# Funatiq/cuclark

Measured on AMD Instinct MI355X. Metric: Mreads/sec (10M x 150bp, k=31), higher is better.
Workload: dtype u64

## Files before the change

cuclark_amd/csrc/mic_device.h:

```cpp
#ifndef MIC_DEVICE_H
#define MIC_DEVICE_H

#include "mic_internal.h"

__device__ __forceinline__ uint32_t bperm(int src_lane, uint32_t v) {
  return (uint32_t)__builtin_amdgcn_ds_bpermute(src_lane << 2, (int)v);
}

template <int CTRL>
__device__ __forceinline__ uint32_t quad_perm(uint32_t v) {
  return (uint32_t)__builtin_amdgcn_update_dpp(0, (int)v, CTRL, 0xF, 0xF, true);
}
#define QP_BCAST0 0x00
#define QP_BCAST1 0x55
#define QP_BCAST3 0xFF
#define QP_XOR1 0xB1
#define QP_XOR2 0x4E

__device__ __forceinline__ uint64_t revcomp_bits(uint64_t x, int k) {
  uint32_t rh = __builtin_bitreverse32((uint32_t)x), rl = __builtin_bitreverse32((uint32_t)(x >> 32));
  rh = ((rh >> 1) & 0x55555555u) | ((rh << 1) & ~0x55555555u);
  rl = ((rl >> 1) & 0x55555555u) | ((rl << 1) & ~0x55555555u);
  return (((uint64_t)~rh << 32) | (uint32_t)~rl) >> (64 - 2 * k);
}

__device__ __forceinline__ uint64_t canonical(uint64_t kmer, int k) {
  uint64_t rc = revcomp_bits(kmer, k);
  return kmer < rc ? kmer : rc;
}

#ifndef MIC_HASH_LITE
#define MIC_HASH_LITE 2
#endif
#ifndef MIC_CHEAP_HASH
#define MIC_CHEAP_HASH 1
#endif
__device__ __forceinline__ uint32_t mmer_order_key_canon(uint64_t u) {
#if MIC_CHEAP_HASH
  const uint32_t hi = (uint32_t)(u >> 32);
  uint32_t h = (uint32_t)u * 0x9E3779B1u ^ (__umul24(hi ^ (hi >> 24), 0xEBCA77u) + 0x27D4EB2Fu);
#else
  uint32_t h = (uint32_t)u * 0x9E3779B1u ^ ((uint32_t)(u >> 32) * 0x85EBCA77u + 0x27D4EB2Fu);
#endif
#if MIC_HASH_LITE & 1
  h *= 0x2C1B3C6Du;
#else
  h ^= h >> 15; h *= 0x2C1B3C6Du;
#endif
  return h;
}

__device__ __forceinline__ uint32_t mmer_order_key(uint64_t x, int m) { return mmer_order_key_canon(canonical(x, m)); }

__device__ __forceinline__ uint32_t mslot_of_key(uint32_t min_key, uint32_t n_slots) {
#if MIC_CHEAP_HASH
  return __umulhi(min_key * 0xC2B2AE3Du, n_slots);
#else
  uint32_t z = min_key * 0xC2B2AE3Du;
  z ^= z >> 15; z *= 0x165667B1u;
  return __umulhi(z, n_slots);
#endif
}

__device__ __forceinline__ uint32_t mslot_of_kmer(uint64_t kmer, int k, int m, uint32_t n_slots) {
  const uint64_t mask = (1ULL << (2 * m)) - 1;
  uint32_t best = 0xFFFFFFFFu;
  for (int j = 0; j + m <= k; ++j) {
    uint32_t h = mmer_order_key((kmer >> (2 * (k - m - j))) & mask, m);
    best = h < best ? h : best;
  }
  return mslot_of_key(best, n_slots);
}

#define MIC_S_CAP 6
#define MIC_S_NEXT 0x100u

#ifndef MIC_S_MOD
#define MIC_S_MOD 1
#endif
__host__ __device__ __forceinline__ int s_tlen(int k, int m) {
  int t = m;
#if MIC_S_MOD
  const int w = k - m + 1;
  while (t - w >= 7) t -= w;
#endif
  return t;
}
__device__ __forceinline__ uint32_t s_torder(uint64_t tv) {
  uint32_t h = __umul24((uint32_t)tv & 0xFFFFFFu, 0x9E3779u) + 0x27D4EB2Fu;
  const uint32_t hi = (uint32_t)(tv >> 24);
  if (hi) h += hi * 0x85EBCA77u + (uint32_t)(tv >> 56) * 0xC2B2AE3Du;
  return h;
}
__device__ __forceinline__ uint32_t s_torder24(uint32_t tv) { return __umul24(tv, 0x9E3779u) + 0x27D4EB2Fu; }
__device__ __forceinline__ uint32_t swap_comp_pairs(uint32_t a, uint32_t b) {
#if defined(__HIP_DEVICE_COMPILE__)
  return (uint32_t)__builtin_amdgcn_bitop3_b32(a, b, 0x55555555u, 0x1B);
#else
  return ~((a & 0x55555555u) | (b & ~0x55555555u));
#endif
}
__device__ __forceinline__ uint32_t revcomp_bits32(uint32_t x, int t) {
#if defined(__HIP_DEVICE_COMPILE__)
  const uint32_t br = __builtin_bitreverse32(x);
  const uint32_t b = (__builtin_constant_p(t) && t < 16) ? br >> (31 - 2 * t) : (br << 1) >> (32 - 2 * t);
  return swap_comp_pairs(br >> (33 - 2 * t), b) & (t >= 16 ? 0xFFFFFFFFu : (1u << (2 * t)) - 1u);
#else
  uint32_t r = __builtin_bitreverse32(x) >> (32 - 2 * t);
  r = ((r >> 1) & 0x55555555u) | ((r << 1) & ~0x55555555u);
  return ~r & (t >= 16 ? 0xFFFFFFFFu : (1u << (2 * t)) - 1u);
#endif
}
template <typename F>
__device__ __forceinline__ void s_sampled(uint64_t K, int k, int m, bool canon, F&& f) {
  const int w = k - m + 1, t = s_tlen(k, m), W = k - t + 1;
  const uint64_t tmask = t >= 32 ? ~0ULL : (1ULL << (2 * t)) - 1;
  uint32_t hmin = 0xFFFFFFFFu, set = 0;
  int p = 0;
  for (int i = 0; i < W; ++i) {
    uint32_t h;
    if (t <= 12) {
      uint32_t tv = (uint32_t)(K >> (2 * (k - t - i))) & (uint32_t)tmask;
      if (canon) { const uint32_t tr = revcomp_bits32(tv, t); tv = tr < tv ? tr : tv; }
      h = s_torder24(tv) >> 5;
    } else {
      uint64_t tv = (K >> (2 * (k - t - i))) & tmask;
      if (canon) { const uint64_t tr = revcomp_bits(tv, t); tv = tr < tv ? tr : tv; }
      h = s_torder(tv) >> 5;
    }
    if (h < hmin) { hmin = h; set = 0; }
    if (h == hmin) set |= 1u << p;
    if (++p == w) p = 0;
  }
  while (set) {
    const int q = __builtin_ctz(set);
    set &= set - 1;
    f(q);
  }
}

__device__ __forceinline__ uint32_t sslot_hash(uint64_t x) {
  const uint32_t hi = (uint32_t)(x >> 32);
  uint32_t h = (uint32_t)x * 0x85EBCA77u + __umul24(hi ^ (hi >> 24), 0xC2B2AFu);
#if !(MIC_HASH_LITE & 2)
  h ^= h >> 15; h *= 0x165667B1u;
#endif
  return h;
}
__device__ __forceinline__ uint32_t sslot_of_x(uint64_t x, uint32_t n_slots) { return __umulhi(sslot_hash(x), n_slots); }

__device__ __forceinline__ uint32_t sslot_of_x32(uint32_t lo, uint32_t hi, uint32_t n_slots) {
  uint32_t h = lo * 0x85EBCA77u + __umul24(hi ^ (hi >> 24), 0xC2B2AFu);
#if !(MIC_HASH_LITE & 2)
  h ^= h >> 15; h *= 0x165667B1u;
#endif
  return __umulhi(h, n_slots);
}

__device__ __forceinline__ uint64_t s_extract(uint32_t w0, uint32_t w1, uint32_t w2, int a, int k) {
  const int s = 2 * a;
  const uint64_t hi = ((uint64_t)w0 << 32) | w1;
  const uint64_t x = (hi << s) | ((uint64_t)w2 >> (32 - s));
  return x >> (64 - 2 * k);
}

template <typename F>
__device__ __forceinline__ void s_candidates(uint64_t c, int k, int m, F&& f) {
  const int w = k - m + 1;
  const uint64_t mask = (1ULL << (2 * m)) - 1;
  const uint64_t rc = revcomp_bits(c, k);
  uint32_t P = 0;
  s_sampled(c, k, m, true, [&](int p) { P |= 1u << p; });
  for (uint32_t left = P; left; left &= left - 1) {
    const int p = __builtin_ctz(left);
    const uint64_t mf = (c >> (2 * (k - m - p))) & mask, mr = revcomp_bits(mf, m);
    if (mf <= mr) f(c, p, mf);
    if (mf >= mr && !(rc == c && ((P >> (w - 1 - p)) & 1u))) f(rc, w - 1 - p, mr);
  }
}

template <typename F>
__device__ __forceinline__ void s_candidates_fwd(uint64_t c, int k, int m, F&& f) {
  const uint64_t mask = (1ULL << (2 * m)) - 1;
  const uint64_t rc = revcomp_bits(c, k);
  for (int strand = 0; strand < 2; ++strand) {
    if (strand && rc == c) break;
    const uint64_t K = strand ? rc : c;
    s_sampled(K, k, m, false, [&](int p) { f(K, p, (K >> (2 * (k - m - p))) & mask); });
  }
}

__device__ __forceinline__ uint32_t s_side_hash(uint64_t K, uint32_t mask) {
  uint64_t x = K * 0x9E3779B97F4A7C15ull;
  x ^= x >> 29;
  x *= 0xBF58476D1CE4E5B9ull;
  return (uint32_t)(x >> 32) >> __builtin_clz(mask | 1u);
}
__device__ inline uint32_t s_side_probe(const uint4* __restrict__ side, uint32_t mask, uint64_t K) {
  uint32_t h = s_side_hash(K, mask);
  for (;;) {
    const uint4 c = side[h];
    if (c.z == 0) return 0;
    if (c.x == (uint32_t)K && c.y == (uint32_t)(K >> 32)) return c.z;
    h = (h + 1) & mask;
  }
}

__device__ inline uint32_t s_probe_read(const uint4* __restrict__ slots, uint32_t n_slots, bool parted, uint32_t slot_lo,
                                        uint32_t slot_cnt, uint64_t K, uint32_t tpos, int k, int m, bool fwd, bool* mine,
                                        const uint4* __restrict__ side = nullptr, uint32_t side_mask = 0) {
  const int w = k - m + 1, t = s_tlen(k, m), W = k - t + 1;
  const uint64_t mask = (1ULL << (2 * m)) - 1;
  const uint64_t tmask = t >= 32 ? ~0ULL : (1ULL << (2 * t)) - 1;
  uint32_t best = 0xFFFFFFFFu; int bi = 0;
  for (int i = 0; i < W; ++i) {
    uint64_t tv = (K >> (2 * (k - t - i))) & tmask;
    if (!fwd) { const uint64_t tr = revcomp_bits(tv, t); tv = tr < tv ? tr : tv; }
    const uint32_t key = (s_torder(tv) & ~31u) | ((tpos + (uint32_t)i) & 31u);
    if (key < best) { best = key; bi = i; }
  }
  const int p = bi % w;
  const uint64_t mf = (K >> (2 * (k - m - p))) & mask;
  const uint64_t mr = fwd ? 0 : revcomp_bits(mf, m);
  const bool rev = !fwd && mr < mf;
  const uint64_t x = rev ? mr : mf;
  const uint64_t Kq = rev ? revcomp_bits(K, k) : K;
  const int j = rev ? w - 1 - p : p;
  uint64_t slot = sslot_of_x(x, n_slots);
  if (parted && (uint32_t)slot - slot_lo >= slot_cnt) { *mine = false; return 0; }
  *mine = true;
  for (;;) {
    const uint32_t* q = (const uint32_t*)(slots + slot * 8);
    for (int e = 0; e < MIC_S_CAP; ++e) {
      if (q[e] != (uint32_t)x) continue;
      const uint32_t pl = q[24 + e];
      if ((pl >> 16) == 0 && side && s_extract(q[6 + 3 * e], q[7 + 3 * e], q[8 + 3 * e], w - 1, m) == x) return s_side_probe(side, side_mask, Kq);
      if (!((pl >> (16 + j)) & 1)) continue;
      if (s_extract(q[6 + 3 * e], q[7 + 3 * e], q[8 + 3 * e], w - 1 - j, k) == Kq) return (pl & 0xFFFFu) + 1;
    }
    if (!(q[30] & MIC_S_NEXT)) return 0;
    slot = q[31];
  }
}

#define MIC_M_N(meta) ((meta) & 0xFFu)
#define MIC_M_DIR 0x100u

#endif
```

cuclark_amd/csrc/mic_kernels.hip:

```cpp
#include "mic_internal.h"
#include "mic_device.h"

#include <stdlib.h>

#ifndef MIC_EXP
#define MIC_EXP 0
#endif
#ifndef MIC_FUNNEL64
#define MIC_FUNNEL64 1
#endif
#ifndef MIC_X
#define MIC_X 0
#endif

namespace {

__device__ __forceinline__ uint4 load_slot_quarter(const uint4* p) {
  typedef unsigned int u4 __attribute__((ext_vector_type(4)));
  u4 t = __builtin_nontemporal_load((const u4*)p);
  return make_uint4(t.x, t.y, t.z, t.w);
}

__device__ __forceinline__ uint64_t kmer_from_dwords(uint32_t d0, uint32_t d1, uint32_t d2, int nt_in_dword, int k) {
  const int s = 2 * nt_in_dword;
// ... 274 lines not shown
        }
        tally2(res0, res1, acc, n_ent, overflow, total, lane);
      }
    }
    finish_read(acc, n_ent, total, overflow, r, a, lane);
  }
}


#define MIC_RMAX 32
#define MIC_MSTRIDE 8
#ifndef MIC_R_SKEW
#define MIC_R_SKEW 2
#endif
#ifndef MIC_R_PIPE
#define MIC_R_PIPE 2
#endif
__device__ __forceinline__ uint32_t staged_at(uint32_t i) { return i * MIC_MSTRIDE + (i >> 3) * MIC_R_SKEW; }
#ifndef MIC_M_SKEW
#define MIC_M_SKEW 0
#endif
__device__ __forceinline__ uint32_t staged_at_m(uint32_t i) { return i * MIC_MSTRIDE + (i >> 3) * MIC_M_SKEW; }

__device__ __forceinline__ void sliding_min3(uint32_t& a0, uint32_t& a1, uint32_t& a2, int w, int lane) {
  auto step = [&](int s) {
    const int src = (lane + s) & 63;
    const bool wrap = lane + s >= 64;
    uint32_t x0 = bperm(src, a0), x1 = bperm(src, a1), x2 = bperm(src, a2);
    uint32_t n0 = wrap ? x1 : x0, n1 = wrap ? x2 : x1, n2 = wrap ? 0xFFFFFFFFu : x2;
    a0 = n0 < a0 ? n0 : a0; a1 = n1 < a1 ? n1 : a1; a2 = n2 < a2 ? n2 : a2;
  };
  int cover = 1;
  while (2 * cover <= w) { step(cover); cover *= 2; }
  if (cover < w) step(w - cover);
}

__device__ __forceinline__ void sliding_min2(uint32_t& a0, uint32_t& a1, int w, int lane) {
  auto step = [&](int s) {
    const int src = (lane + s) & 63;
    const bool wrap = lane + s >= 64;
    uint32_t x0 = bperm(src, a0), x1 = bperm(src, a1);
    uint32_t n0 = wrap ? x1 : x0, n1 = wrap ? 0xFFFFFFFFu : x1;
    a0 = n0 < a0 ? n0 : a0; a1 = n1 < a1 ? n1 : a1;
  };
  int cover = 1;
  while (2 * cover <= w) { step(cover); cover *= 2; }
  if (cover < w) step(w - cover);
}

__device__ __forceinline__ uint32_t row_prefix_min(uint32_t t) {
  uint32_t x;
  x = (uint32_t)__builtin_amdgcn_update_dpp(-1, (int)t, 0x111, 0xF, 0xF, false); t = x < t ? x : t;
  x = (uint32_t)__builtin_amdgcn_update_dpp(-1, (int)t, 0x112, 0xF, 0xF, false); t = x < t ? x : t;
  x = (uint32_t)__builtin_amdgcn_update_dpp(-1, (int)t, 0x114, 0xF, 0xF, false); t = x < t ? x : t;
  x = (uint32_t)__builtin_amdgcn_update_dpp(-1, (int)t, 0x118, 0xF, 0xF, false); t = x < t ? x : t;
  return t;
}

__device__ __forceinline__ uint32_t row_suffix_min(uint32_t t) {
  uint32_t x;
  x = (uint32_t)__builtin_amdgcn_update_dpp(-1, (int)t, 0x101, 0xF, 0xF, false); t = x < t ? x : t;
  x = (uint32_t)__builtin_amdgcn_update_dpp(-1, (int)t, 0x102, 0xF, 0xF, false); t = x < t ? x : t;
  x = (uint32_t)__builtin_amdgcn_update_dpp(-1, (int)t, 0x104, 0xF, 0xF, false); t = x < t ? x : t;
  x = (uint32_t)__builtin_amdgcn_update_dpp(-1, (int)t, 0x108, 0xF, 0xF, false); t = x < t ? x : t;
  asm("" : "+v"(t));
  return t;
}

template <int BANKS>
__device__ __forceinline__ uint32_t with_row_in_front(uint32_t P) {
  const uint32_t f = (uint32_t)__builtin_amdgcn_update_dpp(-1, (int)P, 0x142, 0xE, BANKS, false);
  return f < P ? f : P;
}
__device__ __forceinline__ void sliding_min_rows(uint32_t& a0, uint32_t& a1, uint32_t a2, int W, int lane, int lane_inv) {
  const uint32_t P0 = row_prefix_min(a0), P1 = row_prefix_min(a1), P2 = row_prefix_min(a2);
  if (W > 16 && ((W - 16) & 3) == 0) {
    const uint32_t S0 = row_suffix_min(a0), S1 = row_suffix_min(a1);
    const int s = W - 16, bm = (1 << (s >> 2)) - 1;
    uint32_t Q0, Q1, Q2;
    switch (bm) {
      case 1: Q0 = with_row_in_front<1>(P0); Q1 = with_row_in_front<1>(P1); Q2 = with_row_in_front<1>(P2); break;
      case 3: Q0 = with_row_in_front<3>(P0); Q1 = with_row_in_front<3>(P1); Q2 = with_row_in_front<3>(P2); break;
      case 7: Q0 = with_row_in_front<7>(P0); Q1 = with_row_in_front<7>(P1); Q2 = with_row_in_front<7>(P2); break;
      default: Q0 = with_row_in_front<15>(P0); Q1 = with_row_in_front<15>(P1); Q2 = with_row_in_front<15>(P2); break;
    }
    const uint32_t f0 = __builtin_amdgcn_readlane(P0, 63), f1 = __builtin_amdgcn_readlane(P1, 63);
    const bool head = lane < s;
    const uint32_t h1 = f0 < Q1 ? f0 : Q1, h2 = f1 < Q2 ? f1 : Q2;
    Q1 = head ? h1 : Q1; Q2 = head ? h2 : Q2;
    const int at = (lane_inv << 2) + ((W - 1) << 2);
    const uint32_t z0 = (uint32_t)__builtin_amdgcn_ds_bpermute(at, (int)Q0), z1 = (uint32_t)__builtin_amdgcn_ds_bpermute(at, (int)Q1),
                   z2 = (uint32_t)__builtin_amdgcn_ds_bpermute(at, (int)Q2);
    const bool wz = lane >= 65 - W;
    const uint32_t v0 = wz ? z1 : z0, v1 = wz ? z2 : z1;
    a0 = v0 < S0 ? v0 : S0; a1 = v1 < S1 ? v1 : S1;
    return;
  }
  const uint32_t S0 = row_suffix_min(a0), S1 = row_suffix_min(a1), S2 = row_suffix_min(a2);
  const int at = lane_inv << 2;
  const uint32_t x0 = (uint32_t)__builtin_amdgcn_ds_bpermute(at + 60, (int)P0), x1 = (uint32_t)__builtin_amdgcn_ds_bpermute(at + 60, (int)P1),
                 x2 = (uint32_t)__builtin_amdgcn_ds_bpermute(at + 60, (int)P2);
  const bool wr = lane >= 49;
  const uint32_t n0 = wr ? x1 : x0, n1 = wr ? x2 : x1;
  uint32_t M0 = n0 < S0 ? n0 : S0, M1 = n1 < S1 ? n1 : S1;
  if (W > 16) {
    const uint32_t M2 = x2 < S2 ? x2 : S2;
    const int sh = (W - 16) << 2;
    const uint32_t y0 = (uint32_t)__builtin_amdgcn_ds_bpermute(at + sh, (int)M0), y1 = (uint32_t)__builtin_amdgcn_ds_bpermute(at + sh, (int)M1),
                   y2 = (uint32_t)__builtin_amdgcn_ds_bpermute(at + sh, (int)M2);
    const bool wy = lane >= 80 - W;
    const uint32_t v0 = wy ? y1 : y0, v1 = wy ? y2 : y1;
    M0 = v0 < M0 ? v0 : M0; M1 = v1 < M1 ? v1 : M1;
  }
  a0 = M0; a1 = M1;
}

template <bool CANON>
__device__ __forceinline__ void sampled_positions(uint32_t wd, int ln, int lane_inv, int k, int m, bool past, uint32_t& qa0, uint32_t& qa1) {
  const int w = k - m + 1, t = s_tlen(k, m), W = k - t + 1;
  const uint32_t pb = (uint32_t)lane_inv & 31u;
  uint32_t a0, a1, a2 = 0xFFFFFFFFu;
  if (t <= 16) {
    const int s1 = lane_inv - 1;
    const int ad = (s1 >> 4) << 2;
    const uint32_t tsh = 30u - 2u * (uint32_t)(s1 & 15);
    auto tkey = [&](int h) {
      const uint32_t W0 = (uint32_t)__builtin_amdgcn_ds_bpermute(ad + 16 * h, (int)wd), W1 = (uint32_t)__builtin_amdgcn_ds_bpermute(ad + 16 * h + 4, (int)wd);
      uint32_t tv = __builtin_amdgcn_alignbit(W0, W1, tsh) >> (32 - 2 * t);
      if (CANON) { const uint32_t tr = revcomp_bits32(tv, t); tv = tr < tv ? tr : tv; }
      return ((t <= 12 ? s_torder24(tv) : s_torder(tv)) & ~31u) | pb;
    };
    a0 = tkey(0); a1 = tkey(1);
    if (past) a2 = tkey(2);
  } else {
    auto tkey = [&](int h) {
      const int idx = 4 * h + (lane_inv >> 4);
      const uint32_t d0 = bperm(idx, wd), d1 = bperm(idx + 1, wd), d2 = bperm(idx + 2, wd);
      uint64_t tv = kmer_from_dwords(d0, d1, d2, lane_inv & 15, t);
      if (CANON) { const uint64_t tr = revcomp_bits(tv, t); tv = tr < tv ? tr : tv; }
      return (s_torder(tv) & ~31u) | pb;
    };
    a0 = tkey(0); a1 = tkey(1);
    if (past) a2 = tkey(2);
  }
  if (W >= 16) sliding_min_rows(a0, a1, a2, W, ln, lane_inv);
  else sliding_min3(a0, a1, a2, W, ln);
  uint32_t d0 = (a0 - pb) & 31u, d1 = (a1 - pb) & 31u;
  if (W == 2 * w) { const uint32_t e0 = d0 - (uint32_t)w, e1 = d1 - (uint32_t)w; d0 = e0 < d0 ? e0 : d0; d1 = e1 < d1 ? e1 : d1; }
  else if (W != w) {
    const uint32_t rcp = (1024u + (uint32_t)w - 1u) / (uint32_t)w;
    d0 -= (uint32_t)w * ((d0 * rcp) >> 10); d1 -= (uint32_t)w * ((d1 * rcp) >> 10);
  }
  qa0 = (uint32_t)lane_inv + d0; qa1 = 64u + (uint32_t)lane_inv + d1;
}

#ifndef MIC_SPEC
#define MIC_SPEC 1
#endif
#ifndef MIC_M_WPB
#define MIC_M_WPB 4
#endif
template <int KK, int MM>
__global__ void __launch_bounds__(64 * MIC_M_WPB, 32 / MIC_M_WPB) query_kernel_m(const MicQueryArgs a) {
  __shared__ uint4 s_stage[MIC_M_WPB][MIC_RMAX * MIC_MSTRIDE + (MIC_RMAX / 8 - 1) * MIC_M_SKEW];
  __shared__ uint32_t s_run[MIC_M_WPB][MIC_RMAX];
  __shared__ uint32_t s_ahead[MIC_M_WPB][2][64];
  const int lane = threadIdx.x & 63;
  const int wv = __builtin_amdgcn_readfirstlane(threadIdx.x >> 6);
  uint4* stage = s_stage[wv];
  uint32_t* runslot = s_run[wv];
  const uint32_t wave0 = __builtin_amdgcn_readfirstlane(blockIdx.x * MIC_M_WPB + wv);
  const uint32_t n_waves = gridDim.x * MIC_M_WPB;
  const MicTable& t = a.t;
  const int k = KK ? KK : t.k, m = MM ? MM : t.m, w = k - m + 1;
  const uint4* __restrict__ slots = t.slots;
  const uint16_t* __restrict__ cont = a.cont;
  auto below = [](uint64_t mask) { return (uint32_t)__builtin_amdgcn_mbcnt_hi((uint32_t)(mask >> 32), __builtin_amdgcn_mbcnt_lo((uint32_t)mask, 0u)); };

  uint32_t* ahead0 = s_ahead[wv][0];
  uint32_t* ahead1 = s_ahead[wv][1];
  auto ahead_issue = [&](uint32_t* entry, uint32_t pp_w, uint32_t r_ptr) {
    const uint64_t abase = ((uint64_t)(cont + pp_w)) & ~3ULL;
    const uint32_t rr = r_ptr < a.n_reads ? r_ptr : a.n_reads - 1;
    const uint64_t pbase = (uint64_t)(a.reads_ptr + rr) - 48;
    uint32_t lv = (uint32_t)lane;
    asm volatile("" : "+v"(lv));
    const uint32_t li = lv < 14 ? lv : 0u;
    const uint64_t addr = (li < 12 ? abase : pbase) + 4 * li;
    __builtin_amdgcn_global_load_lds((const __attribute__((address_space(1))) void*)addr,
                                     (__attribute__((address_space(3))) void*)entry, 4, 0, 0);
  };
  auto ahead_take = [&](const uint32_t* entry, uint32_t pp_w, uint32_t& hdr, uint32_t& wword, uint32_t& npp, uint32_t& npe) {
    const uint32_t raw = entry[lane];
    npp = __builtin_amdgcn_readlane(raw, 12); npe = __builtin_amdgcn_readlane(raw, 13);
    const bool odd = (((uint64_t)(cont + pp_w)) >> 1) & 1;
    const uint32_t up = (uint32_t)__builtin_amdgcn_update_dpp(0, (int)raw, 0x101, 0xF, 0xF, true);
    const uint32_t first = __builtin_amdgcn_readfirstlane(raw);
    hdr = odd ? first >> 16 : first & 0xFFFFu;
    wword = odd ? ((up << 16) | (up >> 16)) : ((raw & 0xFFFF0000u) | (up & 0xFFFFu));
  };
  uint32_t cur_pp, cur_pe, cur_hdr, cur_w;
  uint32_t n_pp, n_pe;
  uint32_t ahead_sel;
  {
    const uint32_t r0 = wave0 < a.n_reads ? wave0 : a.n_reads - 1;
    cur_pp = __builtin_amdgcn_readfirstlane(a.reads_ptr[r0]); cur_pe = __builtin_amdgcn_readfirstlane(a.reads_ptr[r0 + 1]);
    ahead_issue(ahead0, cur_pp, wave0 + n_waves);
    asm volatile("s_waitcnt vmcnt(0)" ::: "memory");
    __builtin_amdgcn_wave_barrier();
    ahead_take(ahead0, cur_pp, cur_hdr, cur_w, n_pp, n_pe);
    ahead_issue(ahead1, n_pp, wave0 + 2 * n_waves);
    ahead_sel = 1;
  }
  for (uint32_t r = wave0; r < a.n_reads; r += n_waves) {
    uint32_t pp = cur_pp;
    const uint32_t pe = cur_pe;
    RowAcc acc; acc.label1 = 0; acc.count = 0;
    uint32_t n_ent = 0, overflow = 0, total = 0;
    bool first_part = true;

    while (pp < pe) {
      const uint32_t plen = __builtin_amdgcn_readfirstlane(first_part ? cur_hdr : (uint32_t)cont[pp]);
      const bool ahead_ok = first_part;
      first_part = false;
      if (plen == 0) break;
      const uint32_t first = pp + 1;
      pp = first + (plen + 7) / 8;
      if (plen < (uint32_t)k) continue;
      const uint32_t nk = plen - k + 1;
      const uint32_t cend = pp;
      for (uint32_t base = 0; base < nk; base += 128) {
        const uint32_t wd = window_word_w(cont, first, cend, base, lane, ahead_ok && base == 0, cur_w);
        uint64_t c[2]; bool act[2]; uint32_t hk0, hk1, hk2;
        const bool past = nk - base > (uint32_t)(129 - w);
        const bool tail_path = w <= 16;
        uint32_t tail = 0xFFFFFFFFu;
#pragma unroll
        for (int h = 0; h < 2; ++h) {
          const int idx = 4 * h + (lane >> 4);
          uint32_t d0 = bperm(idx, wd), d1 = bperm(idx + 1, wd), d2 = bperm(idx + 2, wd);
          uint64_t kmer = kmer_from_dwords(d0, d1, d2, lane & 15, k);
          const uint64_t rck = revcomp_bits(kmer, k);
          c[h] = kmer < rck ? kmer : rck;
          act[h] = base + 64 * h + lane < nk;
          if (t.sharded) {
            uint64_t kp = (uint64_t)__builtin_amdgcn_kernarg_segment_ptr();
            asm volatile("" : "+s"(kp));
            const __attribute__((address_space(4))) MicQueryArgs* kc = (const __attribute__((address_space(4))) MicQueryArgs*)kp;
            MicDiv dv; dv.d = kc->t.div.d; dv.magic = kc->t.div.magic; dv.shift = kc->t.div.shift; dv.add = kc->t.div.add;
            const uint64_t s_lo = kc->t.shard_start, s_hi = kc->t.shard_end;
            uint64_t q = mic_div(c[h], dv);
            uint64_t rem = c[h] - q * dv.d;
            act[h] = act[h] && rem >= s_lo && rem < s_hi;
          }
          const uint64_t mf = kmer >> (2 * (k - m)), mr = rck & ((1ULL << (2 * m)) - 1);
          uint32_t key = mmer_order_key_canon(mf < mr ? mf : mr);
          if (h == 0) hk0 = key; else hk1 = key;
          if (h == 1 && tail_path && past) {
            const uint64_t tf = kmer & ((1ULL << (2 * m)) - 1), tr = rck >> (2 * (k - m));
            const uint32_t tk = mmer_order_key_canon(tf < tr ? tf : tr);
            tail = row_prefix_min(lane >= 65 - w ? tk : 0xFFFFFFFFu);
          }
        }
        if (tail_path) {
          sliding_min2(hk0, hk1, w, lane);
          hk1 = tail < hk1 ? tail : hk1;
        } else {
          hk2 = 0xFFFFFFFFu;
          if (past) {
            const int idx = 8 + (lane >> 4);
            uint32_t d0 = bperm(idx, wd), d1 = bperm(idx + 1, wd), d2 = bperm(idx + 2, wd);
            uint64_t mm = kmer_from_dwords(d0, d1, d2, lane & 15, m);
            hk2 = lane < w - 1 ? mmer_order_key(mm, m) : 0xFFFFFFFFu;
          }
          sliding_min3(hk0, hk1, hk2, w, lane);
        }
        uint32_t sl0 = act[0] ? mslot_of_key(hk0, (uint32_t)t.n_main) : 0xFFFFFFFFu;
        uint32_t sl1 = act[1] ? mslot_of_key(hk1, (uint32_t)t.n_main) : 0xFFFFFFFFu;
        uint32_t res0 = 0, res1 = 0, res2 = 0;

        auto level = [&](uint32_t s0_, uint32_t s1_, uint64_t k0_, uint64_t k1_, uint32_t& o0_, uint32_t& o1_, uint32_t& y0_, uint32_t& y1_) {
          uint32_t p0 = bperm((lane + 63) & 63, s0_), p1 = bperm((lane + 63) & 63, s1_);
          uint32_t last0 = bperm(63, s0_);
          if (lane == 0) { p0 = 0xFFFFFFFFu; p1 = last0; }
          const bool f0 = s0_ != 0xFFFFFFFFu && s0_ != p0, f1 = s1_ != 0xFFFFFFFFu && s1_ != p1;
          const uint64_t b0 = __ballot(f0), b1 = __ballot(f1);
          const uint32_t R0 = __popcll(b0), R = R0 + __popcll(b1);
          const uint32_t rid0 = below(b0) + (f0 ? 1u : 0u) - 1, rid1 = R0 + below(b1) + (f1 ? 1u : 0u) - 1;
          y0_ = 0xFFFFFFFFu; y1_ = 0xFFFFFFFFu;
          for (uint32_t rbase = 0; rbase < R; rbase += MIC_RMAX) {
            __builtin_amdgcn_wave_barrier();
            if (f0 && rid0 - rbase < MIC_RMAX) runslot[rid0 - rbase] = s0_;
            if (f1 && rid1 - rbase < MIC_RMAX) runslot[rid1 - rbase] = s1_;
            __builtin_amdgcn_wave_barrier();
            const uint32_t nrun = R - rbase < MIC_RMAX ? R - rbase : MIC_RMAX;
            uint32_t sidx[MIC_RMAX / 8];
#pragma unroll
            for (int i = 0; i < MIC_RMAX / 8; ++i) sidx[i] = runslot[8 * i + (lane >> 3)];
#pragma unroll
            for (int i = 0; i < MIC_RMAX / 8; ++i) {
              if (8u * i >= nrun) break;
              if (8u * i + (lane >> 3) < nrun)
                __builtin_amdgcn_global_load_lds((const __attribute__((address_space(1))) void*)(slots + (uint64_t)sidx[i] * 8 + (lane & 7)),
                                                 (__attribute__((address_space(3))) void*)(stage + (64 + MIC_M_SKEW) * i), 16, 0, 0);
            }
            asm volatile("s_waitcnt vmcnt(0)" ::: "memory");
// ... 303 lines not shown
                if (m1) hit1 = (p1 & 0xFFFFu) + 1;
                {
                  const bool cr0 = same0 && (p0 >> 16) == 0, cr1 = same1 && (p1 >> 16) == 0;
                  if (__ballot(cr0) | __ballot(cr1)) {
                    uint64_t kp = (uint64_t)__builtin_amdgcn_kernarg_segment_ptr();
                    asm volatile("" : "+s"(kp));
                    const __attribute__((address_space(4))) MicQueryArgs* kc = (const __attribute__((address_space(4))) MicQueryArgs*)kp;
                    const uint4* side = kc->t.side; const uint32_t smask = kc->t.side_mask;
                    const uint64_t mm = (1ULL << (2 * m)) - 1;
                    if (side && cr0 && s_extract(a0, b0, c0, w - 1, m) == ((ko[0] >> (2 * ao[0])) & mm)) hit0 = s_side_probe(side, smask, ko[0]);
                    if (side && cr1 && s_extract(a1, b1, c1, w - 1, m) == ((ko[1] >> (2 * ao[1])) & mm)) hit1 = s_side_probe(side, smask, ko[1]);
                  }
                }
                more0 = same0 && !m0 && e0 < 5; more1 = same1 && !m1 && e1 < 5;
                e0 += more0 ? 1u : 0u; e1 += more1 ? 1u : 0u;
                if (!(__ballot(more0) | __ballot(more1))) break;
              }
              if (v0) { o0_ = hit0; y0_ = 0xFFFFFFFFu; }
              if (v1) { o1_ = hit1; y1_ = 0xFFFFFFFFu; }
              const bool n0 = v0 && !hit0 && (mz0 & MIC_S_NEXT), n1 = v1 && !hit1 && (mz1 & MIC_S_NEXT);
              if (__ballot(n0) | __ballot(n1)) {
                if (n0 && q0[5] <= t0) y0_ = q0[31];
                if (n1 && q1[5] <= t1) y1_ = q1[31];
              }
            }
          }
        };
        while (__ballot(sl0 != 0xFFFFFFFFu) | __ballot(sl1 != 0xFFFFFFFFu)) {
          uint32_t nx0, nx1;
          level(sl0, sl1, res0, res1, nx0, nx1);
          sl0 = nx0; sl1 = nx1;
        }
        tally2(res0, res1, acc, n_ent, overflow, total, lane);
      }
    }
    uint32_t t_hdr, t_pp, t_pe;
    asm volatile("s_waitcnt vmcnt(0)" ::: "memory");
    __builtin_amdgcn_wave_barrier();
    ahead_take(ahead_sel ? ahead1 : ahead0, n_pp, t_hdr, t_pp, t_pe);
    __builtin_amdgcn_wave_barrier();
    {
      uint64_t kp = (uint64_t)__builtin_amdgcn_kernarg_segment_ptr();
      asm volatile("" : "+s"(kp));
      const __attribute__((address_space(4))) MicQueryArgs* kc = (const __attribute__((address_space(4))) MicQueryArgs*)kp;
      struct { uint32_t* results; uint32_t* rows; uint32_t* flagged; uint32_t row_words, flagged_cap; } fa;
      fa.results = kc->results; fa.rows = kc->rows; fa.flagged = kc->flagged; fa.row_words = kc->row_words; fa.flagged_cap = kc->flagged_cap;
      finish_read(acc, n_ent, total, overflow, r, fa, lane);
    }
    ahead_issue(ahead_sel ? ahead0 : ahead1, t_pp, r + 3 * n_waves);
    ahead_sel ^= 1;
    cur_pp = n_pp; cur_pe = n_pe; cur_hdr = t_hdr; n_pp = t_pp; n_pe = t_pe;
  }
}


__device__ __forceinline__ uint64_t wballot(bool p) { return __builtin_amdgcn_ballot_w64(p); }

static_assert(MIC_RMAX <= 32, "tally_counts sums the first two rows of lanes");
#define MIC_R_CROWDED (-16)
__device__ __forceinline__ void tally_counts(uint32_t lab1, uint32_t cnt, RowAcc& acc, uint32_t& n_ent, uint32_t& overflow,
                                             uint32_t& total, int lane) {
  uint64_t mm = wballot(lab1 != 0);
  while (mm) {
    const uint32_t l1 = __builtin_amdgcn_readlane(lab1, __builtin_ctzll(mm));
    const bool mine = lab1 == l1;
    mm &= ~wballot(mine);
    const uint32_t c = mine ? cnt : 0u;
    uint32_t sum = 0;
    {
      uint32_t v = c;
      v += (uint32_t)__builtin_amdgcn_update_dpp(0, (int)v, 0x111, 0xF, 0xF, true);
      v += (uint32_t)__builtin_amdgcn_update_dpp(0, (int)v, 0x112, 0xF, 0xF, true);
      v += (uint32_t)__builtin_amdgcn_update_dpp(0, (int)v, 0x114, 0xF, 0xF, true);
      v += (uint32_t)__builtin_amdgcn_update_dpp(0, (int)v, 0x118, 0xF, 0xF, true);
      sum = __builtin_amdgcn_readlane(v, 15) + __builtin_amdgcn_readlane(v, 31);
    }
    total += sum;
    row_add(acc, n_ent, overflow, l1, sum, lane);
  }
}

template <int KK, int MM, bool FWD, bool PART>
__global__ void __launch_bounds__(64 * MIC_M_WPB, 32 / MIC_M_WPB) query_kernel_r(const MicQueryArgs a) {
  __shared__ uint4 s_stage[MIC_M_WPB][MIC_RMAX * MIC_MSTRIDE + (MIC_RMAX / 8 - 1) * MIC_R_SKEW];
  __shared__ uint16_t s_rec[MIC_M_WPB][132];
  __shared__ uint32_t s_ahead[MIC_M_WPB][2][64];
  __shared__ uint32_t s_part[PART ? MIC_M_WPB : 1][2];
  const int lane = threadIdx.x & 63;
  const int wv = __builtin_amdgcn_readfirstlane(threadIdx.x >> 6);
  uint4* stage = s_stage[wv];
  uint16_t* rec = s_rec[wv];
  const uint32_t wave0 = __builtin_amdgcn_readfirstlane(blockIdx.x * MIC_M_WPB + wv);
  const uint32_t n_waves = gridDim.x * MIC_M_WPB;
  const MicTable& t = a.t;
  if (PART) { if (lane == 0) { s_part[wv][0] = t.slot_lo; s_part[wv][1] = t.slot_cnt; } __builtin_amdgcn_wave_barrier(); }
  const int k = KK ? KK : t.k, m = MM ? MM : t.m, ctx = k - m;
  const uint4* __restrict__ slots = t.slots;
  const uint16_t* __restrict__ cont = a.cont;
  auto below = [](uint64_t mask) { return (uint32_t)__builtin_amdgcn_mbcnt_hi((uint32_t)(mask >> 32), __builtin_amdgcn_mbcnt_lo((uint32_t)mask, 0u)); };

  uint32_t* ahead0 = s_ahead[wv][0];
  uint32_t* ahead1 = s_ahead[wv][1];
  auto ahead_issue = [&](uint32_t* entry, uint32_t pp_w, uint32_t r_ptr) {
    const uint64_t abase = ((uint64_t)(cont + pp_w)) & ~3ULL;
    const uint32_t rr = r_ptr < a.n_reads ? r_ptr : a.n_reads - 1;
    const uint64_t pbase = (uint64_t)(a.reads_ptr + rr) - 48;
    int ln = lane;
    asm volatile("" : "+v"(ln));
    if (ln < 12)
      __builtin_amdgcn_global_load_lds((const __attribute__((address_space(1))) void*)((const uint32_t*)abase + lane),
                                       (__attribute__((address_space(3))) void*)entry, 4, 0, 0);
    uint64_t pb = pbase + 48;
    asm volatile("" : "+s"(pb));
    if (ln < 2)
      __builtin_amdgcn_global_load_lds((const __attribute__((address_space(1))) void*)((const uint32_t*)pb + lane),
                                       (__attribute__((address_space(3))) void*)(entry + 12), 4, 0, 0);
  };
  auto ahead_take = [&](const uint32_t* entry, uint32_t pp_w, uint32_t& hdr, uint32_t& npp, uint32_t& npe) {
    const uint32_t raw = entry[lane];
    npp = __builtin_amdgcn_readlane(raw, 12); npe = __builtin_amdgcn_readlane(raw, 13);
    const bool odd = (((uint64_t)(cont + pp_w)) >> 1) & 1;
    const uint32_t first = __builtin_amdgcn_readfirstlane(raw);
    hdr = odd ? first >> 16 : first & 0xFFFFu;
  };
  auto ahead_word = [&](const uint32_t* entry, uint32_t pp_w) {
    const uint32_t raw = entry[lane];
    const bool odd = (((uint64_t)(cont + pp_w)) >> 1) & 1;
    const uint32_t up = (uint32_t)__builtin_amdgcn_update_dpp(0, (int)raw, 0x101, 0xF, 0xF, true);
    return __builtin_amdgcn_perm(up, raw, odd ? 0x05040706u : 0x03020504u);
  };
  uint32_t cur_pp, cur_pe, cur_hdr, n_pp, n_pe, ahead_sel;
  {
    const uint32_t r0 = wave0 < a.n_reads ? wave0 : a.n_reads - 1;
    cur_pp = __builtin_amdgcn_readfirstlane(a.reads_ptr[r0]); cur_pe = __builtin_amdgcn_readfirstlane(a.reads_ptr[r0 + 1]);
    ahead_issue(ahead0, cur_pp, wave0 + n_waves);
    asm volatile("s_waitcnt vmcnt(0)" ::: "memory");
    __builtin_amdgcn_wave_barrier();
    ahead_take(ahead0, cur_pp, cur_hdr, n_pp, n_pe);
    ahead_issue(ahead1, n_pp, wave0 + 2 * n_waves);
    ahead_sel = 1;
  }
  constexpr bool PIPE = KK != 0 && (MIC_R_PIPE >= 2 || (MIC_R_PIPE == 1 && FWD));
  struct Round {
    uint32_t G0, G1, G2, cur;
    int jmax, jmin, remaining;
  };
  auto front = [&](const uint32_t first, const uint32_t cend, const uint32_t base, const uint32_t nk, const bool use_ahead, uint32_t& wd_out) __attribute__((always_inline)) -> uint32_t {
    int ln = lane;
    asm volatile("" : "+v"(ln));
    const uint32_t wd = use_ahead ? ahead_word(ahead_sel ? ahead0 : ahead1, cur_pp)
                                  : window_word_w(cont, first, cend, base, ln, false, 0u);
    wd_out = wd;
    const uint32_t n_act = nk - base < 128u ? nk - base : 128u;
    const bool past = n_act + (uint32_t)(k - s_tlen(k, m)) >= 129u;
    uint32_t qa0, qa1;
    sampled_positions<!FWD>(wd, ln, lane, k, m, past, qa0, qa1);
    qa0 = (uint32_t)lane < n_act ? qa0 : 0xFFu;
    qa1 = 64u + (uint32_t)lane < n_act ? qa1 : 0xFFu;
    const uint32_t last0 = __builtin_amdgcn_readlane(qa0, 63);
    uint32_t p0 = (uint32_t)__builtin_amdgcn_update_dpp(-1, (int)qa0, 0x138, 0xF, 0xF, false);
    uint32_t p1 = (uint32_t)__builtin_amdgcn_update_dpp((int)last0, (int)qa1, 0x138, 0xF, 0xF, false);
    const bool f0 = qa0 != p0, f1 = qa1 != p1;
    const uint64_t b0 = wballot(f0), b1 = wballot(f1);
    const uint32_t R0 = __popcll(b0), R = R0 + __popcll(b1) - (n_act < 128u ? 1u : 0u);
    __builtin_amdgcn_wave_barrier();
    if (f0) rec[below(b0)] = (uint16_t)(qa0 | ((uint32_t)lane << 8));
    if (f1) rec[R0 + below(b1)] = (uint16_t)(qa1 | ((64u + (uint32_t)lane) << 8));
    if (__builtin_expect(n_act == 128u, 0)) {
      asm volatile("" ::: "memory");
      if (ln == 0) rec[R] = (uint16_t)(128u << 8);
    }
    __builtin_amdgcn_wave_barrier();
    return R;
  };
  const uint32_t xsh = (64u - 2u * (uint32_t)k) & 31u;
  auto region_x = [&](uint32_t A0, uint32_t A1, uint32_t& lo, uint32_t& hi) {
    if (k > 16) {
      lo = __builtin_amdgcn_alignbit(A0, A1, xsh) & (m >= 16 ? 0xFFFFFFFFu : (1u << ((2 * m) & 31)) - 1u);
      hi = m > 16 ? (A0 >> xsh) & ((1u << ((2 * m - 32) & 31)) - 1u) : 0u;
    } else {
      const uint64_t x = ((((uint64_t)A0 << 32) | A1) << (2 * ctx)) >> (64 - 2 * m);
      lo = (uint32_t)x; hi = (uint32_t)(x >> 32);
    }
  };
  auto setup = [&](const uint32_t wd, const uint32_t rbase, const uint32_t R, Round& L, uint32_t& nrun_out) __attribute__((always_inline)) {
    const uint32_t nrun = R - rbase < MIC_RMAX ? R - rbase : MIC_RMAX;
    nrun_out = nrun;
    const bool vr = (uint32_t)lane < nrun;
    const uint32_t ri = vr ? rbase + (uint32_t)lane : 0u;
    const uint32_t rc0 = rec[ri], rc1 = rec[ri + 1];
    const int qa = (int)(rc0 & 255u), i0 = (int)(rc0 >> 8);
    const int n = (int)(rc1 >> 8) - i0;
    const int s1 = qa - ctx - 1;
    const int D = s1 >> 4;
    const uint32_t tsh = 30u - 2u * (uint32_t)(s1 & 15);
    const int a0 = D << 2;
    const uint32_t W0 = (uint32_t)__builtin_amdgcn_ds_bpermute(a0, (int)wd), W1 = (uint32_t)__builtin_amdgcn_ds_bpermute(a0 + 4, (int)wd),
                   W2 = (uint32_t)__builtin_amdgcn_ds_bpermute(a0 + 8, (int)wd), W3 = (uint32_t)__builtin_amdgcn_ds_bpermute(a0 + 12, (int)wd);
    uint32_t G0 = __builtin_amdgcn_alignbit(W0, W1, tsh), G1 = __builtin_amdgcn_alignbit(W1, W2, tsh), G2 = __builtin_amdgcn_alignbit(W2, W3, tsh);
    uint32_t key, xhi;
    region_x(G0, G1, key, xhi);
    bool rev = false;
    if (!FWD) {
      const uint32_t sh = 96u - 2u * (uint32_t)(k + ctx);
      const uint32_t r0 = __builtin_bitreverse32(G2), r1 = __builtin_bitreverse32(G1), r2 = __builtin_bitreverse32(G0);
      uint32_t q0, q1, q2;
      if (KK != 0 && sh != 0) {
        q0 = swap_comp_pairs(__builtin_amdgcn_alignbit(r0, r1, 33u - sh), __builtin_amdgcn_alignbit(r0, r1, 31u - sh));
        q1 = swap_comp_pairs(__builtin_amdgcn_alignbit(r1, r2, 33u - sh), __builtin_amdgcn_alignbit(r1, r2, 31u - sh));
        q2 = swap_comp_pairs(r2 << (sh - 1u), r2 << (sh + 1u));
      } else {
        q0 = sh ? __builtin_amdgcn_alignbit(r0, r1, 32u - sh) : r0;
        q1 = sh ? __builtin_amdgcn_alignbit(r1, r2, 32u - sh) : r1;
        q2 = r2 << sh;
        q0 = swap_comp_pairs(q0 >> 1, q0 << 1); q1 = swap_comp_pairs(q1 >> 1, q1 << 1); q2 = swap_comp_pairs(q2 >> 1, q2 << 1);
      }
      uint32_t kr, hr;
      region_x(q0, q1, kr, hr);
      rev = hr < xhi || (hr == xhi && kr < key);
      G0 = rev ? q0 : G0; G1 = rev ? q1 : G1; G2 = rev ? q2 : G2;
      key = rev ? kr : key; xhi = rev ? hr : xhi;
    }
    const int jmaxf = qa - i0, jminf = jmaxf - n + 1;
    const int jmax = rev ? ctx - jminf : jmaxf, jmin = rev ? ctx - jmaxf : jminf;
    uint32_t cur = vr ? sslot_of_x32(key, xhi, (uint32_t)t.n_main) : 0xFFFFFFFFu;
    bool mine = vr;
    if (PART) {
      mine = vr && cur - s_part[wv][0] < s_part[wv][1];
      cur = mine ? cur : 0xFFFFFFFFu;
    }
    L.G0 = G0; L.G1 = G1; L.G2 = G2; L.cur = cur;
    L.jmax = jmax; L.jmin = jmin; L.remaining = mine ? n : 0;
  };
  auto issue = [&](const uint32_t cur, const uint32_t nrun) __attribute__((always_inline)) {
    uint32_t sidx[MIC_RMAX / 8];
    int ln = lane;
    asm volatile("" : "+v"(ln));
    __builtin_amdgcn_wave_barrier();
    if (ln < MIC_RMAX) ((uint32_t*)stage)[lane] = cur;
    __builtin_amdgcn_wave_barrier();
    uint32_t so = (uint32_t)(uintptr_t)(__attribute__((address_space(3))) void*)stage;
    asm volatile("" : "+s"(so));
#pragma unroll
    for (int i = 0; i < MIC_RMAX / 8; ++i) sidx[i] = ((const uint32_t*)stage)[8 * i + (lane >> 3)];
#pragma unroll
    for (int i = 0; i < MIC_RMAX / 8; ++i) {
      if (8u * i >= nrun) break;
      if (sidx[i] != 0xFFFFFFFFu)
        __builtin_amdgcn_global_load_lds((const __attribute__((address_space(1))) void*)(slots + (uint64_t)sidx[i] * 8 + (lane & 7)),
                                         (__attribute__((address_space(3))) void*)(uintptr_t)(so + 16u * (64 + MIC_R_SKEW) * (uint32_t)i), 16, 0, 0);
    }
  };
  auto consume = [&](Round& L, RowAcc& acc, uint32_t& n_ent, uint32_t& overflow, uint32_t& total, uint32_t& cg) __attribute__((always_inline)) {
    const uint32_t G0 = L.G0, G1 = L.G1, G2 = L.G2;
    uint32_t key, xhi_;
    region_x(G0, G1, key, xhi_);
    const int jmax = L.jmax, jmin = L.jmin;
    uint32_t cur = L.cur;
    int remaining = L.remaining;
    bool again = false;
    do {
      if (again) issue(cur, MIC_RMAX);
      again = true;
      asm volatile("s_waitcnt vmcnt(0)" ::: "memory");
      __builtin_amdgcn_wave_barrier();
      const bool vl = cur != 0xFFFFFFFFu;
      const uint32_t* q = (const uint32_t*)(stage + (vl ? staged_at((uint32_t)lane) : 0));
      const uint4 ka = *(const uint4*)q;
      const uint2 kb = *(const uint2*)(q + 4);
      uint32_t e = (ka.x < key) + (ka.y < key) + (ka.z < key) + (ka.w < key) + (kb.x < key) + (kb.y < key);
      const uint32_t mz = q[30];
      bool more = vl && e < 6;
      e = e < 5 ? e : 5;
      for (;;) {
        uint32_t e3 = e + (e << 1);
        asm volatile("" : "+v"(e3));
        uint32_t g = q[e], S0 = q[6 + e3], S1 = q[7 + e3], S2 = q[8 + e3], pl = q[24 + e];
        asm volatile("" : "+v"(S2));
        const bool same = more && g == key;
        const uint32_t d0 = G0 ^ S0, d1 = G1 ^ S1, d2 = G2 ^ S2;
        const bool mineq = k > 16
                               ? ((d0 & ((1u << ((32 - 2 * ctx) & 31)) - 1u)) | (d1 >> xsh)) == 0
                               : (((((uint64_t)d0 << 32) | d1) << (2 * ctx)) >> (64 - 2 * m)) == 0;
        const uint32_t dl = d0 >> (32 - 2 * ctx);
        const uint32_t dr = k > 16 ? __builtin_amdgcn_alignbit(d1, d2, xsh)
                                        : (uint32_t)((((((uint64_t)d0 << 32) | d1)) << ((2 * k) & 63)) >> 32);
        const int left = __builtin_ctz(dl | (1u << (2 * ctx))) >> 1;
        const int right = __builtin_clz(dr | (1u << (31 - 2 * ctx))) >> 1;
        const int hi = left < jmax ? left : jmax, lo = ctx - right > jmin ? ctx - right : jmin;
        const uint32_t range = ((2u << (hi & 31)) - 1u) & (~0u << (lo & 31));
        const uint32_t hits = (same && mineq) ? (uint32_t)__popc((pl >> 16) & range) : 0u;
#if !(MIC_X & 1)
        remaining = (same && mineq && (pl >> 16) == 0) ? MIC_R_CROWDED : remaining;
#endif
        const uint32_t lab_new = (pl & 0xFFFFu) + 1u;
        tally_counts(hits ? lab_new : 0u, hits, acc, n_ent, overflow, total, lane);
        remaining -= (int)hits;
        more = same && remaining > 0 && e < 5;
        e += more ? 1u : 0u;
        if (!wballot(more)) break;
      }
      const bool nx = vl && remaining > 0 && (mz & MIC_S_NEXT);
      cur = 0xFFFFFFFFu;
      if (wballot(nx)) { if (nx && q[5] <= key) cur = q[31]; }
    } while (wballot(cur != 0xFFFFFFFFu));
    if (!(MIC_X & 2) && __builtin_expect(wballot(remaining <= MIC_R_CROWDED) != 0, 0)) {
// ... 589 lines not shown
```

Measured before the change: 2050.

## Add specialized k=31,m=20 front end computing three positions per lane

Adds a specialized sampled-position path for k=31, m=20 in which each lane handles three consecutive k-mer positions instead of two strided ones. Each lane extracts one 16-nt window, builds the three 8-mer keys and their canonical forms from one bit-reversal, and forms the sliding minimum with a short bpermute tree. Record ranks come from chained mbcnt over three ballots. This is meant to cut the permute, shuffle and ALU cost of minimizer selection, at the price of a hard-coded path that must exactly match the generic results, including the n_act==128 terminator that this path no longer writes.

```diff
diff --git a/cuclark_amd/csrc/mic_device.h b/cuclark_amd/csrc/mic_device.h
--- a/cuclark_amd/csrc/mic_device.h
+++ b/cuclark_amd/csrc/mic_device.h
@@ -111,6 +111,7 @@
   return ~r & (t >= 16 ? 0xFFFFFFFFu : (1u << (2 * t)) - 1u);
 #endif
 }
+#include "mic_front3.h"
 template <typename F>
 __device__ __forceinline__ void s_sampled(uint64_t K, int k, int m, bool canon, F&& f) {
   const int w = k - m + 1, t = s_tlen(k, m), W = k - t + 1;
diff --git a/cuclark_amd/csrc/mic_front3.h b/cuclark_amd/csrc/mic_front3.h
--- /dev/null
+++ b/cuclark_amd/csrc/mic_front3.h
@@ -0,0 +1,88 @@
+#ifndef MIC_FRONT3_H
+#define MIC_FRONT3_H
+
+#include <stdint.h>
+
+#if defined(__HIPCC__)
+#define F3_FN __host__ __device__ __forceinline__
+#else
+#define F3_FN static inline
+#endif
+
+#define F3_K 31
+#define F3_M 20
+#define F3_T 8
+#define F3_WIN (F3_K - F3_T + 1)
+#define F3_WM (F3_K - F3_M + 1)
+
+F3_FN int f3_dword(int a) { return (3 * a - 1) >> 4; }
+F3_FN uint32_t f3_shift(int a) { return 30u - 2u * (uint32_t)((3 * a - 1) & 15); }
+F3_FN uint32_t f3_funnel(uint32_t hi, uint32_t lo, uint32_t sh) { return (uint32_t)((((uint64_t)hi << 32) | lo) >> sh); }
+
+F3_FN uint32_t f3_tmer(uint32_t X, int j) { return (X << (2 * j)) >> 16; }
+F3_FN uint32_t f3_rc10(uint32_t X) {
+  uint32_t r = 0;
+  for (int i = 0; i < 10; ++i) r |= (3u - ((X >> (30 - 2 * i)) & 3u)) << (2 * i);
+  return r;
+}
+F3_FN uint32_t f3_tmer_rc(uint32_t Y, int j) { return (Y >> (2 * j)) & 0xFFFFu; }
+F3_FN uint32_t f3_key(uint32_t tv, uint32_t pos) { return (((tv & 0xFFFFFFu) * 0x9E3779u + 0x27D4EB2Fu) & ~31u) | (pos & 31u); }
+
+F3_FN uint32_t f3_min(uint32_t a, uint32_t b) { return a < b ? a : b; }
+F3_FN uint32_t f3_min3(uint32_t a, uint32_t b, uint32_t c) { return f3_min(f3_min(a, b), c); }
+F3_FN void f3_combine(uint32_t k2, uint32_t e12, uint32_t m4, uint32_t x1, uint32_t y, uint32_t z, uint32_t k0n, uint32_t e01n,
+                      uint32_t& r0, uint32_t& r1, uint32_t& r2) {
+  r0 = f3_min(m4, z);
+  const uint32_t M7 = f3_min3(x1, y, z);
+  r1 = f3_min3(e12, M7, k0n);
+  r2 = f3_min3(k2, M7, e01n);
+}
+F3_FN uint32_t f3_sampled(uint32_t r, uint32_t pos) {
+  const uint32_t d = (r - pos) & 31u, e = d - (uint32_t)F3_WM;
+  return pos + f3_min(d, e);
+}
+F3_FN uint32_t f3_rank(uint32_t below0, uint32_t below1, uint32_t below2, bool f0, bool f1, int j) {
+  return below0 + below1 + below2 + (j > 0 && f0 ? 1u : 0u) + (j > 1 && f1 ? 1u : 0u);
+}
+F3_FN uint16_t f3_record(uint32_t q, uint32_t pos) { return (uint16_t)(q | (pos << 8)); }
+
+#if !defined(__HIP_DEVICE_COMPILE__)
+static inline uint32_t f3_model(const uint32_t wd[64], uint32_t n_act, bool canon, uint32_t q[192], uint16_t rec[132]) {
+  uint32_t s[192];
+  uint32_t k0[64], k2[64], T[64], e12[64], e01[64], m2[64], m4[64];
+  for (int a = 0; a < 64; ++a) {
+    const int D = f3_dword(a);
+    const uint32_t X = f3_funnel(wd[D & 63], wd[(D + 1) & 63], f3_shift(a)), Y = f3_rc10(X);
+    uint32_t kk[3];
+    for (int j = 0; j < 3; ++j) {
+      uint32_t tv = f3_tmer(X, j);
+      if (canon) tv = f3_min(tv, f3_tmer_rc(Y, j));
+      kk[j] = f3_key(tv, (uint32_t)(3 * a + j));
+    }
+    k0[a] = kk[0]; k2[a] = kk[2];
+    T[a] = f3_min3(kk[0], kk[1], kk[2]); e12[a] = f3_min(kk[1], kk[2]); e01[a] = f3_min(kk[0], kk[1]);
+  }
+  for (int a = 0; a < 64; ++a) m2[a] = f3_min(T[a], T[(a + 1) & 63]);
+  for (int a = 0; a < 64; ++a) m4[a] = f3_min(m2[a], m2[(a + 2) & 63]);
+  bool f[192];
+  for (int a = 0; a < 64; ++a) {
+    uint32_t r[3];
+    f3_combine(k2[a], e12[a], m4[a], T[(a + 1) & 63], m2[(a + 2) & 63], m4[(a + 4) & 63], k0[(a + 8) & 63], e01[(a + 8) & 63], r[0], r[1], r[2]);
+    for (int j = 0; j < 3; ++j) {
+      const uint32_t pos = (uint32_t)(3 * a + j);
+      s[pos] = f3_sampled(r[j], pos);
+      q[pos] = pos < n_act ? s[pos] : ~0u;
+    }
+  }
+  for (int i = 0; i < 192; ++i) f[i] = i == 0 || q[i] != q[i - 1];
+  uint32_t below[3] = {0, 0, 0}, total = 0;
+  for (int a = 0; a < 64; ++a) {
+    for (int j = 0; j < 3; ++j)
+      if (f[3 * a + j]) { rec[f3_rank(below[0], below[1], below[2], f[3 * a], f[3 * a + 1], j)] = f3_record(s[3 * a + j], (uint32_t)(3 * a + j)); ++total; }
+    for (int j = 0; j < 3; ++j) below[j] += f[3 * a + j];
+  }
+  return total - 1u;
+}
+#endif
+
+#endif
diff --git a/cuclark_amd/csrc/mic_kernels.hip b/cuclark_amd/csrc/mic_kernels.hip
--- a/cuclark_amd/csrc/mic_kernels.hip
+++ b/cuclark_amd/csrc/mic_kernels.hip
@@ -450,6 +450,42 @@
     d0 -= (uint32_t)w * ((d0 * rcp) >> 10); d1 -= (uint32_t)w * ((d1 * rcp) >> 10);
   }
   qa0 = (uint32_t)lane_inv + d0; qa1 = 64u + (uint32_t)lane_inv + d1;
+}
+
+template <bool CANON>
+__device__ __forceinline__ void sampled_positions3(uint32_t wd, int lane_inv, uint32_t n_act, uint32_t& p0, uint32_t& s0, uint32_t& s1, uint32_t& s2,
+                                                    uint32_t& q0, uint32_t& q1, uint32_t& q2) {
+  const int at = lane_inv << 2;
+  const int ad = f3_dword(lane_inv) << 2;
+  const uint32_t tsh = f3_shift(lane_inv);
+  p0 = 3u * (uint32_t)lane_inv;
+  const uint32_t np0 = 0u - p0;
+  const uint32_t W0 = (uint32_t)__builtin_amdgcn_ds_bpermute(ad, (int)wd), W1 = (uint32_t)__builtin_amdgcn_ds_bpermute(ad + 4, (int)wd);
+  const uint32_t X = __builtin_amdgcn_alignbit(W0, W1, tsh);
+  uint32_t t0 = f3_tmer(X, 0), t1 = f3_tmer(X, 1), t2 = f3_tmer(X, 2);
+  if (CANON) {
+    const uint32_t br = __builtin_bitreverse32(X);
+    const uint32_t Y = swap_comp_pairs(br >> 1, br << 1);
+    t0 = f3_min(t0, f3_tmer_rc(Y, 0)); t1 = f3_min(t1, f3_tmer_rc(Y, 1)); t2 = f3_min(t2, f3_tmer_rc(Y, 2));
+  }
+  auto key = [](uint32_t tv, uint32_t pos) { return (uint32_t)__builtin_amdgcn_bitop3_b32(s_torder24(tv), pos, 31u, 0xD8); };
+  const uint32_t k0 = key(t0, p0), k1 = key(t1, p0 + 1u), k2 = key(t2, p0 + 2u);
+  const uint32_t T = f3_min3(k0, k1, k2), e12 = f3_min(k1, k2), e01 = f3_min(k0, k1);
+  const uint32_t x1 = (uint32_t)__builtin_amdgcn_ds_bpermute(at + 4, (int)T);
+  const uint32_t m2 = f3_min(T, x1);
+  const uint32_t y = (uint32_t)__builtin_amdgcn_ds_bpermute(at + 8, (int)m2);
+  const uint32_t m4 = f3_min(m2, y);
+  const uint32_t z = (uint32_t)__builtin_amdgcn_ds_bpermute(at + 16, (int)m4);
+  const uint32_t k0n = (uint32_t)__builtin_amdgcn_ds_bpermute(at + 32, (int)k0), e01n = (uint32_t)__builtin_amdgcn_ds_bpermute(at + 32, (int)e01);
+  uint32_t r0, r1, r2;
+  f3_combine(k2, e12, m4, x1, y, z, k0n, e01n, r0, r1, r2);
+  auto sampled = [&](uint32_t r, uint32_t j) {
+    const uint32_t d = (r + np0 - j) & 31u, e = d - (uint32_t)F3_WM;
+    return f3_min(d, e) + p0 + j;
+  };
+  const int nv = (int)(n_act + np0);
+  s0 = sampled(r0, 0u); s1 = sampled(r1, 1u); s2 = sampled(r2, 2u);
+  q0 = nv > 0 ? s0 : ~0u; q1 = nv > 1 ? s1 : ~0u; q2 = nv > 2 ? s2 : ~0u;
 }
 
 #ifndef MIC_SPEC
@@ -1059,6 +1095,24 @@
                                   : window_word_w(cont, first, cend, base, ln, false, 0u);
     wd_out = wd;
     const uint32_t n_act = nk - base < 128u ? nk - base : 128u;
+    if constexpr (KK == F3_K && MM == F3_M) {
+      uint32_t p0, s0, s1, s2, q0, q1, q2;
+      sampled_positions3<!FWD>(wd, lane, n_act, p0, s0, s1, s2, q0, q1, q2);
+      const uint32_t pv = (uint32_t)__builtin_amdgcn_update_dpp(-1, (int)q2, 0x138, 0xF, 0xF, false);
+      const bool f0 = q0 != pv, f1 = q1 != q0, f2 = q2 != q1;
+      const uint64_t b0 = wballot(f0), b1 = wballot(f1), b2 = wballot(f2);
+      const uint32_t R = __popcll(b0) + __popcll(b1) + __popcll(b2) - 1u;
+      uint32_t c = __builtin_amdgcn_mbcnt_hi((uint32_t)(b0 >> 32), __builtin_amdgcn_mbcnt_lo((uint32_t)b0, 0u));
+      c = __builtin_amdgcn_mbcnt_hi((uint32_t)(b1 >> 32), __builtin_amdgcn_mbcnt_lo((uint32_t)b1, c));
+      c = __builtin_amdgcn_mbcnt_hi((uint32_t)(b2 >> 32), __builtin_amdgcn_mbcnt_lo((uint32_t)b2, c));
+      __builtin_amdgcn_wave_barrier();
+      const uint32_t c1 = c + (f0 ? 1u : 0u), c2 = c1 + (f1 ? 1u : 0u);
+      if (f0) rec[c] = f3_record(s0, p0);
+      if (f1) rec[c1] = f3_record(s1, p0 + 1u);
+      if (f2) rec[c2] = f3_record(s2, p0 + 2u);
+      __builtin_amdgcn_wave_barrier();
+      return R;
+    }
     const bool past = n_act + (uint32_t)(k - s_tlen(k, m)) >= 129u;
     uint32_t qa0, qa1;
     sampled_positions<!FWD>(wd, ln, lane, k, m, past, qa0, qa1);
```

After: 2118, median of 6. 3.3% higher.
